# buaacyw/GaussianEditor

Hardware: AMD Instinct MI355X
Metric: train iters/sec (fwd+bwd of one 1080p view per GPU + grad all-reduce), 1M Gaussians @1080p (higher is better)
Workload: dtype f32; 1 GPU; synth-v1 1000000 Gaussians SH3 (M=16, s0=0.01), 1920x1080, ring-v1 8 views, one view per GPU (BASELINE.json configs[3] shape; configs[1] bicycle.ply is not available offline); gaussians=1000000, width=1920, height=1080, views_per_rank=1, parallelism=dp1-views, view_pipeline=False, tile_bounds=reference, fast_exp=False, grad_exchange=direct, grad_exchange_route=local, grad_rows=every row of every gradient written every iteration, num_rendered=0, visible=0, pixel_instances=0, sort_key_bits=45

## Files before the change

gaussianeditor_amd/_native.py:

```python
from __future__ import annotations

import ctypes
import os
from ctypes import c_float, c_int, c_int64, c_size_t, c_uint, c_void_p, POINTER

_HERE = os.path.dirname(os.path.abspath(__file__))
LIB_PATH = os.environ.get("GSR_LIBRARY_PATH") or os.path.join(_HERE, "libgsr_hip.so")
GSR_ABI_VERSION = 6

_P = c_void_p
ACC_ROW, ACC_MEAN2D, ACC_OPACITY, ACC_CONIC, ACC_COLOR, ACC_DEPTH = 16, 0, 3, 4, 8, 11


class AdamTensor(ctypes.Structure):
    _fields_ = [("param", _P), ("grad", _P), ("exp_avg", _P), ("exp_avg_sq", _P), ("anchor", _P), ("numel", c_int64),
                ("row_len", ctypes.c_int32), ("masked", ctypes.c_int32), ("lr", ctypes.c_double), ("anchor_scale", c_float)]


class DenseGrads(ctypes.Structure):
    _fields_ = [("means3D", _P), ("scales", _P), ("rotations", _P), ("means2D", _P), ("opacities", _P), ("sh", _P)]


class AppendTensor(ctypes.Structure):
    _fields_ = [("src", _P), ("ext", _P), ("dst", _P), ("row_bytes", c_int64)]
# ... 48 lines not shown
    "gsr_append_rows": (c_int, [_P, c_int64, c_int64, c_int, POINTER(AppendTensor)]),
    "gsr_adam_step": (c_int, [_P, c_int, POINTER(AdamTensor), c_int64, ctypes.c_double, ctypes.c_double, ctypes.c_double, _P,
                            _P]),
    "gsr_adam_step_rows": (c_int, [_P, c_int, POINTER(AdamTensor), c_int64, ctypes.c_double, ctypes.c_double, ctypes.c_double, _P,
                            _P, _P]),
    "gsr_mark_visible": (c_int, [_P, c_int, _P, _P, _P, _P]),
    "gsr_trace_weights": (c_int, [_P, c_int, c_int64, c_int, c_int, c_int, _P, _P, _P, _P, _P, _P, c_uint]),
    "gsr_debug_export_geom": (c_int, [_P, c_int, _P, _P, _P, _P, _P, _P, _P]),
    "gsr_debug_cov3d": (c_int, [_P, c_int, _P, c_float, _P, _P]),
    "gsr_debug_export_binning": (c_int, [_P, c_int, c_int64, c_int, c_int, _P, _P, _P, _P]),
    "gsr_debug_blend_backward_profile": (c_int, [_P, c_int, c_int64, c_int, c_int, _P, _P, _P, _P, _P, _P, _P,
                                                 c_int64, POINTER(c_int64)]),
    "gsr_debug_blend_forward_profile": (c_int, [_P, c_int, c_int64, c_int, c_int, _P, _P, _P, _P, _P, _P, _P, c_int64,
                                                POINTER(c_int64)]),
    "gsr_debug_export_image": (c_int, [_P, c_int, c_int, _P, _P, _P, _P]),
}

_lib = None


class GsrError(RuntimeError):

    def __init__(self, fn: str, status: int, message: str, hip_error: int = 0):
        self.status = status
        self.hip_error = hip_error
        extra = f" (hipError_t {hip_error})" if hip_error else ""
        super().__init__(f"{fn} failed: {message} [status {status}]{extra}")


def lib() -> ctypes.CDLL:
# ... 29 lines not shown
```

gaussianeditor_amd/csrc/gsr_binning.hip:

```cpp
#include <stdlib.h>

#include "gsr_kernels.h"

namespace gsr {

__device__ __forceinline__ int f2i_sat(float v) {
  if (!(v == v)) return 0;
  if (v >= 2147483648.0f) return 2147483647;
  if (v <= -2147483648.0f) return (-2147483647 - 1);
  return (int)v;
}

constexpr int RBITS = 8;
constexpr int RBINS = 1 << RBITS;

template <class K, int TH, bool WEIGHTED = false>
__global__ void __launch_bounds__(TH) sort_hist_kernel(const K* __restrict__ keys, int64_t n, int shift,
                                                                uint32_t mask, uint32_t* __restrict__ hist,
                                                                uint32_t nblocks, const uint4* __restrict__ publish_src,
                                                                uint32_t publish_count, uint32_t* __restrict__ publish_dst,
                                                                uint32_t publish_seq, const uint32_t* __restrict__ rect32) {
  __shared__ uint32_t h[RBINS];
  __shared__ uint32_t hw[WEIGHTED ? RBINS : 1];
  if (publish_dst != nullptr && blockIdx.x == nblocks) {
    __shared__ unsigned long long psum[TH / 64];
    __shared__ uint32_t pmax[TH / 64], pinv[TH / 64];
    __shared__ unsigned long long pgrp[TH / 64];
    unsigned long long sum = 0, gsum = 0;
    uint32_t kmax = 0, kinv = 0;
    constexpr int PUB_UNROLL = 8;
    for (uint32_t base = threadIdx.x; base < publish_count; base += TH * PUB_UNROLL) {
      uint4 v[PUB_UNROLL];
#pragma unroll
      for (int u = 0; u < PUB_UNROLL; ++u) v[u] = publish_src[min(base + (uint32_t)u * TH, publish_count - 1u)];
#pragma unroll
      for (int u = 0; u < PUB_UNROLL; ++u) {
        if (base + (uint32_t)u * TH < publish_count) {
          sum += v[u].x;
          gsum += v[u].w;
          kmax = max(kmax, v[u].y);
          kinv = max(kinv, v[u].z);
        }
      }
    }
#pragma unroll
    for (int d = 32; d >= 1; d >>= 1) {
      sum += __shfl_xor(sum, d, 64);
      gsum += __shfl_xor(gsum, d, 64);
      kmax = max(kmax, (uint32_t)__shfl_xor((int)kmax, d, 64));
      kinv = max(kinv, (uint32_t)__shfl_xor((int)kinv, d, 64));
    }
    if (lane_id() == 0) {
      psum[threadIdx.x >> 6] = sum;
      pgrp[threadIdx.x >> 6] = gsum;
      pmax[threadIdx.x >> 6] = kmax;
      pinv[threadIdx.x >> 6] = kinv;
    }
    __syncthreads();
    if (threadIdx.x == 0) {
      for (int w = 1; w < TH / 64; ++w) {
        sum += psum[w];
        gsum += pgrp[w];
        kmax = max(kmax, pmax[w]);
        kinv = max(kinv, pinv[w]);
      }
      publish_dst[0] = (uint32_t)sum;
      publish_dst[1] = (uint32_t)(sum >> 32);
      publish_dst[GEOM_HDR_KEYMAX] = kmax;
      publish_dst[GEOM_HDR_KEYINVMAX] = kinv;
      publish_dst[GEOM_HDR_GROUPS] = (uint32_t)gsum;
      publish_dst[GEOM_HDR_GROUPS + 1] = (uint32_t)(gsum >> 32);
      __threadfence_system();
      __hip_atomic_store(publish_dst + GEOM_HDR_FINAL, publish_seq, __ATOMIC_RELEASE, __HIP_MEMORY_SCOPE_SYSTEM);
    }
    return;
  }
  if (threadIdx.x < RBINS) {
    h[threadIdx.x] = 0;
    if (WEIGHTED) hw[threadIdx.x] = 0;
  }
  __syncthreads();
  const int64_t base = (int64_t)blockIdx.x * SORT_KPB;
  uint32_t kv[(SORT_KPB / TH)], rv[WEIGHTED ? (SORT_KPB / TH) : 1];
#pragma unroll
  for (int i = 0; i < (SORT_KPB / TH); ++i) {
    const int64_t k = base + (int64_t)i * TH + threadIdx.x;
    kv[i] = (uint32_t)keys[k < n ? k : n - 1];
    if (WEIGHTED) rv[i] = rect32[k < n ? k : n - 1];
  }
// ... 315 lines not shown
    const int j = i * TH + (int)threadIdx.x;
    if (j < nvalid) {
      const uint32_t kk = LAST ? 0u : skey[j];
      const uint32_t d = LAST ? (uint32_t)sdig[j] : (kk >> shift) & mask;
      const uint32_t first = lexcl[d];
      const uint32_t pos = gbase[d] + ((uint32_t)j - first);
      keys_out[pos] = LAST ? wgbase[d] + (spre[j] - spre[first]) : kk;
      vals_out[pos] = sval[j];
      rect_out[pos] = srect[j];
    }
  }
}

template <int TH>
static void depth_sort_grouped_th(hipStream_t s, int P, const Geom& g, int p0, int p1, bool last, uint32_t* publish_dst,
                                  uint32_t publish_seq) {
  const int64_t n = P;
  const uint32_t nblocks = (uint32_t)((n + SORT_KPB - 1) / SORT_KPB);
  const uint32_t npart = (uint32_t)((P + GAUSS_BLOCK - 1) / GAUSS_BLOCK);
  uint32_t* const hdr = reinterpret_cast<uint32_t*>(g.total);
  for (int p = p0; p < p1; ++p) {
    const int cur = p & 1, shift = 8 * p;
    const bool pub = p == p0 && publish_dst != nullptr, fin = last && p == p1 - 1;
    const dim3 gh(nblocks + (pub ? 1u : 0u)), gs(nblocks), bt(TH), bh(1024);
    if (fin)
      hipLaunchKernelGGL((sort_hist_kernel<uint32_t, 1024, true>), gh, bh, 0, s, (const uint32_t*)g.dkey[cur], n, shift, 255u, g.ghist,
                         nblocks, pub ? g.k1_partials : nullptr, npart, pub ? publish_dst : nullptr, publish_seq,
                         (const uint32_t*)g.drect[cur]);
    else
      hipLaunchKernelGGL((sort_hist_kernel<uint32_t, 1024, false>), gh, bh, 0, s, (const uint32_t*)g.dkey[cur], n, shift, 255u, g.ghist,
                         nblocks, pub ? g.k1_partials : nullptr, npart, pub ? publish_dst : nullptr, publish_seq,
                         (const uint32_t*)nullptr);
    hipLaunchKernelGGL(sort_scan_kernel, dim3(fin ? 2 * RBINS : RBINS), dim3(SORT_THREADS), 0, s, g.ghist, g.gbin_total, nblocks);
#define GSR_DEPTH_SCATTER(LASTP, IOTAP)                                                                                          \
  hipLaunchKernelGGL((depth_scatter_kernel<LASTP, IOTAP, TH>), gs, bt, 0, s, (const uint32_t*)g.dkey[cur],                       \
                     (const uint32_t*)g.dval[cur], (const uint32_t*)g.drect[cur], (const uint2*)g.rect, g.dkey[cur ^ 1],         \
                     g.dval[cur ^ 1], g.drect[cur ^ 1], n, shift, 255u, (const uint32_t*)g.ghist, (const uint32_t*)g.gbin_total, \
                     nblocks, hdr, (uint32_t)(cur ^ 1))
    if (fin && p == 0) GSR_DEPTH_SCATTER(true, true);
    else if (fin) GSR_DEPTH_SCATTER(true, false);
    else if (p == 0) GSR_DEPTH_SCATTER(false, true);
    else GSR_DEPTH_SCATTER(false, false);
#undef GSR_DEPTH_SCATTER
  }
}
hipError_t launch_depth_passes_grouped(hipStream_t s, int P, const Geom& g, int p0, int p1, bool last, uint32_t* publish_dst,
                                       uint32_t publish_seq) {
  if ((uint32_t)(((int64_t)P + SORT_KPB - 1) / SORT_KPB) <= SORT_WIDE_MAX_BLOCKS)
    depth_sort_grouped_th<1024>(s, P, g, p0, p1, last, publish_dst, publish_seq);
  else
    depth_sort_grouped_th<SORT_THREADS>(s, P, g, p0, p1, last, publish_dst, publish_seq);
  return hipGetLastError();
}

__global__ void __launch_bounds__(GAUSS_BLOCK) sorted_block_sums_kernel(int P, int gx, int sgx, const uint32_t* __restrict__ order,
                                                                       const uint2* __restrict__ rect,
                                                                       uint32_t* __restrict__ wh_sorted,
                                                                       uint32_t* __restrict__ org_sorted,
                                                                       uint32_t* __restrict__ block_sums,
                                                                       uint32_t* __restrict__ hdr, uint32_t final_buf) {
  __shared__ uint32_t smem[GAUSS_BLOCK / 64 + 1];
  if (blockIdx.x == 0 && threadIdx.x == 0) hdr[GEOM_HDR_FINAL] = final_buf;
  const int i = (int)(blockIdx.x * GAUSS_BLOCK + threadIdx.x);
  const uint2 rc = i < P ? rect[order[i]] : make_uint2(0u, 0u);
  const uint32_t w = rc.y & 0xffffu, h = rc.y >> 16, x0 = rc.x & 0xffffu, y0 = rc.x >> 16;
  uint32_t n = w * h, org = y0 * (uint32_t)gx + x0;
// ... 797 lines not shown
```

gaussianeditor_amd/csrc/gsr_capi.hip:

```cpp
#include <math.h>
#include <stdlib.h>
#include <string.h>

#include <chrono>
#include <mutex>


#include "gsr_kernels.h"

using namespace gsr;

namespace {
thread_local int g_last_hip_error = 0;
inline int hip_fail(hipError_t e) {
  g_last_hip_error = (int)e;
  return GSR_ERR_HIP;
}
#define GSR_HIP(expr)                          \
  do {                                         \
    hipError_t _e = (expr);                    \
    if (_e != hipSuccess) return hip_fail(_e); \
  } while (0)

struct HostSlot {
  uint32_t* words = nullptr;
  uint32_t* dev_words = nullptr;
  uint32_t seq = 0;
  int device = -1;
  HostSlot* next_free = nullptr;
};
constexpr int MAX_DEV = 64;
std::mutex g_pool_mutex;
HostSlot* g_pool_free[MAX_DEV] = {};

struct ThreadSlots {
  HostSlot* held[MAX_DEV] = {};
  ~ThreadSlots() {
    std::lock_guard<std::mutex> lock(g_pool_mutex);
    for (int d = 0; d < MAX_DEV; ++d)
      if (held[d] != nullptr) {
        held[d]->next_free = g_pool_free[d];
        g_pool_free[d] = held[d];
      }
// ... 131 lines not shown
}
inline bool geom_is_forward_only(const void* geom) {
  std::lock_guard<std::mutex> lock(g_notes_mutex);
  const GeomNote& n = g_notes[note_slot(geom)];
  return n.geom == geom && n.forward_only;
}

inline int bin_legacy(int W, int H) {
  static const bool forced = [] {
    const char* e = getenv("GSR_BIN_LEGACY");
    return e != nullptr && e[0] == '1';
  }();
  const int gx = (W + TILE - 1) / TILE, gy = (H + TILE - 1) / TILE;
  return (forced || group_count(W, H) > GROUP_MAX || gx > RECT32_EDGE || gy > RECT32_EDGE) ? 1 : 0;
}
inline int checkpoint_chunks(int64_t R, int W, int H) {
  static const int env = [] {
    const char* e = getenv("GSR_CK_CHUNKS");
    const char* d = getenv("GSR_CK_DEBUG");
    int c = e != nullptr ? atoi(e) : -1;
    if (c > 0 && c < 4 && !(d != nullptr && d[0] == '1')) c = 4;
    return c > 1024 ? 1024 : c;
  }();
  if (env >= 0) return env;
  static const int64_t env_min_list = [] {
    const char* e = getenv("GSR_CK_MIN_LIST");
    return (int64_t)(e != nullptr && atoi(e) > 0 ? atoi(e) : 0);
  }();
  const int64_t T = (int64_t)((W + TILE - 1) / TILE) * ((H + TILE - 1) / TILE);
  const int64_t min_list = env_min_list > 0 ? env_min_list : (T <= 4096 ? 1200 : 2048);
// ... 160 lines not shown
  a.opacities = opacities; a.shs = shs; a.cov3D_precomp = cov3D_precomp; a.colors_precomp = colors_precomp;
  a.viewmatrix = viewmatrix; a.projmatrix = projmatrix; a.campos = campos;
  a.W = W; a.H = H; a.tan_fovx = tan_fovx; a.tan_fovy = tan_fovy;
  a.focal_y = H / (2.0f * tan_fovy);
  a.focal_x = W / (2.0f * tan_fovx);
  a.gx = (W + TILE - 1) / TILE; a.gy = (H + TILE - 1) / TILE;
  a.skip_color = skip_color;
  a.forward_only = (flags & GSR_FLAG_FORWARD_ONLY) ? 1 : 0;
  a.tile_bounds = (flags & GSR_FLAG_TILE_BOUNDS_ALPHA) ? 1 : 0;
  a.radii = radii;
  a.g = carve_geom(geom, P);
  note_geom(geom, a.forward_only != 0);
  GSR_HIP(launch_preprocess(s, a));
  const uint32_t seq = ++slot->seq ? slot->seq : ++slot->seq;
  *seq_out = seq;
  if (bin_legacy(W, H)) GSR_HIP(launch_depth_passes(s, P, a.g, 0, 2, slot->dev_words, seq));
  else GSR_HIP(launch_depth_passes_grouped(s, P, a.g, 0, 2, false, slot->dev_words, seq));
  return GSR_OK;
}

int preprocess_end_impl(hipStream_t s, int P, int W, int H, void* geom, HostSlot* slot, uint32_t seq, int64_t counts_host[2]) {
  GSR_HIP(wait_for_slot(slot, seq, s));
  const Geom g = carve_geom(geom, P);
  const int gx = (W + TILE - 1) / TILE;
  const int legacy = bin_legacy(W, H);
  const uint32_t* w = slot->words;
  const uint64_t total = (uint64_t)w[0] | ((uint64_t)w[1] << 32);
  const uint32_t kmax = w[GEOM_HDR_KEYMAX], kinv = w[GEOM_HDR_KEYINVMAX];
  const uint32_t kmin = ~kinv;
  int nbits = 0;
  for (uint32_t d = total ? (kmax ^ kmin) : 0u; d; d >>= 1) ++nbits;
  if (legacy) {
    const int passes = nbits <= 16 ? 2 : (nbits + 7) / 8;
    if (passes > 2) GSR_HIP(launch_depth_passes(s, P, g, 2, passes));
    GSR_HIP(launch_depth_finish(s, P, g, passes, gx, 0));
  } else {
    const int passes = nbits <= 24 ? 3 : 4;
    GSR_HIP(launch_depth_passes_grouped(s, P, g, 2, passes, true));
  }
  if (total >= (1ull << 31)) return GSR_ERR_TOO_MANY;
  counts_host[0] = (int64_t)total;
  counts_host[1] = legacy ? 0 : (int64_t)((uint64_t)w[GEOM_HDR_GROUPS] | ((uint64_t)w[GEOM_HDR_GROUPS + 1] << 32));
  return GSR_OK;
}
}

int gsr_preprocess(void* stream, int P, int D, int M, const float* means3D, const float* scales, float scale_modifier,
                   const float* rotations, const float* opacities, const float* shs, const float* cov3D_precomp,
                   const float* colors_precomp, const float* viewmatrix, const float* projmatrix, const float* campos,
                   int W, int H, float tan_fovx, float tan_fovy, int prefiltered, int skip_color, unsigned flags,
// ... 584 lines not shown
}

int gsr_debug_export_binning(void* stream, int P, int64_t R, int W, int H, const void* geom, const void* binning,
                             uint64_t* keys, uint32_t* point_list) {
  if (R <= 0) return GSR_OK;
  if (!binning || !geom) return GSR_ERR_BAD_ARGUMENT;
  const Geom g = carve_geom(const_cast<void*>(geom), P);
  const Binning b = carve_binning_view(binning, R, W, H);
  hipStream_t s = (hipStream_t)stream;
  if (keys) GSR_HIP(launch_export_keys(s, R, W, H, b, g, keys));
  if (point_list)
    GSR_HIP(hipMemcpyAsync(point_list, b.point_list, sizeof(uint32_t) * (size_t)R, hipMemcpyDeviceToDevice, s));
  return GSR_OK;
}

int gsr_debug_export_image(void* stream, int W, int H, const void* image, uint32_t* ranges, float* final_T,
                           uint32_t* n_contrib) {
  if (!image || W <= 0 || H <= 0) return GSR_ERR_BAD_ARGUMENT;
  const Image im = carve_image(const_cast<void*>(image), W, H);
  hipStream_t s = (hipStream_t)stream;
  const size_t T = (size_t)((W + TILE - 1) / TILE) * ((H + TILE - 1) / TILE), N = (size_t)W * H;
  if (ranges) GSR_HIP(hipMemcpyAsync(ranges, im.ranges, sizeof(uint2) * T, hipMemcpyDeviceToDevice, s));
  if (final_T) GSR_HIP(hipMemcpyAsync(final_T, im.final_T, sizeof(float) * N, hipMemcpyDeviceToDevice, s));
  if (n_contrib) GSR_HIP(hipMemcpyAsync(n_contrib, im.n_contrib, sizeof(uint32_t) * N, hipMemcpyDeviceToDevice, s));
  return GSR_OK;
}

}
```

gaussianeditor_amd/csrc/gsr_common.h:

```cpp
#pragma once

#include <hip/hip_runtime.h>
#include <stddef.h>
#include <stdint.h>

#include "../../include/gsr.h"

namespace gsr {

constexpr int TILE = 16;
constexpr int QUAD = 8;
constexpr int WAVE = 64;
constexpr int GAUSS_BLOCK = 256;
constexpr uint32_t ACC_ROW = GSR_ACC_ROW, ACC_MEAN2D = GSR_ACC_MEAN2D, ACC_OPACITY = GSR_ACC_OPACITY, ACC_CONIC = GSR_ACC_CONIC,
                   ACC_COLOR = GSR_ACC_COLOR, ACC_DEPTH = GSR_ACC_DEPTH;
static_assert(ACC_ROW == 16 && ACC_MEAN2D == 0 && ACC_OPACITY == 3 && ACC_CONIC == 4 && ACC_COLOR == 8, "float4-aligned column groups");
static_assert(ACC_DEPTH == ACC_COLOR + 3, "the depth column is the .w of the colour group: K8+K9 reads it with the colour");
constexpr int GROUP_SHIFT = 3;
constexpr int GROUP_EDGE = 1 << GROUP_SHIFT;
constexpr int GROUP_TILES = GROUP_EDGE * GROUP_EDGE;
constexpr int GROUP_MAX = 2048;
constexpr uint32_t GROUP_PAD = 0xffffffffu;

__host__ __device__ inline size_t align_up(size_t v, size_t a = 256) { return (v + a - 1) / a * a; }
// ... 11 lines not shown
  uint4* k1_partials;
  uint32_t* dkey[2];
  uint32_t* dval[2];
  uint32_t* drect[2];
  uint32_t* ghist;
  uint32_t* gbin_total;
  size_t bytes;
};

constexpr int GEOM_HDR_SLOTS = 64;
constexpr int GEOM_HDR_SLOT_WORDS = 32;
constexpr int GEOM_HDR_KEYMAX = 2;
constexpr int GEOM_HDR_KEYINVMAX = 3;
constexpr int GEOM_HDR_FINAL = 4;
constexpr int GEOM_HDR_GROUPS = 5;
constexpr int GEOM_HDR_BYTES = GEOM_HDR_SLOTS * GEOM_HDR_SLOT_WORDS * 4;

__host__ __device__ inline Geom carve_geom(void* base, int P) {
  char* p = (char*)base;
  const size_t nb = ((size_t)P + GAUSS_BLOCK - 1) / GAUSS_BLOCK;
  Geom g;
  size_t off = 0;
  g.total = (uint64_t*)(p + off);      off += align_up(GEOM_HDR_BYTES);
  g.k1_partials = (uint4*)(p + off);   off += align_up(sizeof(uint4) * nb);
  g.rec0 = (float4*)(p + off);         off += align_up(sizeof(float4) * (size_t)P);
  g.rec1 = (float4*)(p + off);         off += align_up(sizeof(float4) * (size_t)P);
  g.rec2 = (float4*)(p + off);         off += align_up(sizeof(float4) * (size_t)P);
  for (int i = 0; i < 3; ++i) { g.dcol[i] = (float*)(p + off); off += align_up(sizeof(float) * 3 * (size_t)P); }
  g.rect = (uint2*)(p + off);          off += align_up(sizeof(uint2) * (size_t)P);
  g.clamped = (uint8_t*)(p + off);     off += align_up((size_t)P);
// ... 307 lines not shown
```

gaussianeditor_amd/csrc/gsr_kernels.h:

```cpp
#pragma once
#include "gsr_common.h"

namespace gsr {

struct PreArgs {
  int P, D, M;
  const float* means3D;
  const float* scales;
  float scale_modifier;
  const float* rotations;
  const float* opacities;
  const float* shs;
  const float* cov3D_precomp;
  const float* colors_precomp;
  const float* viewmatrix;
  const float* projmatrix;
  const float* campos;
  int W, H;
  float tan_fovx, tan_fovy, focal_x, focal_y;
  int gx, gy;
  int skip_color;
  int forward_only;
  int tile_bounds;
  int32_t* radii;
// ... 89 lines not shown
int64_t view_message_words_host(int64_t P, int64_t cap);
hipError_t launch_view_message_header(hipStream_t s, int64_t P, const float* campos, const uint32_t* block_off,
                                      const uint64_t* total, float* msg);
hipError_t launch_view_messages_accumulate(hipStream_t s, int64_t P, int D, int M, int n_views, const float* messages,
                                           int64_t stride_words, int64_t cap, const float* means3D, float* const dense[6],
                                           uint8_t* row_valid);
const uint32_t* compact_block_off_ptr(void* workspace, int64_t P);
hipError_t launch_export_cov3d(hipStream_t s, int P, const float* scales, float scale_modifier, const float* rotations,
                               float* cov3D);
hipError_t launch_export_geom(hipStream_t s, int P, const Geom& g, float* means2D, float* depths, float* rgb,
                              float* conic_opacity, uint32_t* tiles_touched, uint8_t* clamped);
hipError_t launch_depth_passes(hipStream_t s, int P, const Geom& g, int p0, int p1, uint32_t* publish_dst = nullptr,
                               uint32_t publish_seq = 0);
hipError_t launch_depth_finish(hipStream_t s, int P, const Geom& g, int passes, int gx, int sgx);
hipError_t launch_depth_passes_grouped(hipStream_t s, int P, const Geom& g, int p0, int p1, bool last,
                                       uint32_t* publish_dst = nullptr, uint32_t publish_seq = 0);
hipError_t launch_export_keys(hipStream_t s, int64_t R, int W, int H, const Binning& b, const Geom& g, uint64_t* keys);
hipError_t launch_binning(hipStream_t s, int P, int64_t R, int W, int H, const Geom& g, const Binning& b, const Image& im);
size_t knn_workspace_bytes(int P);
hipError_t launch_knn(hipStream_t s, int P, const float* points, void* workspace, float* out);
hipError_t launch_near_points(hipStream_t s, int n_ref, const float* ref, int n_query, const float* query, float thresh,
                              void* workspace, uint8_t* near, float* nn_dist);
size_t compact_workspace_bytes(int64_t P);
hipError_t launch_compact_plan(hipStream_t s, int64_t P, const uint8_t* keep, void* workspace);
const uint64_t* compact_total_ptr(void* workspace, int64_t P);
hipError_t launch_compact_apply(hipStream_t s, int64_t P, const uint8_t* keep, void* workspace, int nt,
                                const gsr_compact_tensor* tensors, int64_t limit = -1);
hipError_t launch_append_rows(hipStream_t s, int64_t P, int64_t n, int nt, const gsr_append_tensor* tensors);
hipError_t launch_adam_step(hipStream_t s, int nt, const gsr_adam_tensor* tensors, long long step, double beta1,
                            double beta2, double eps, const uint8_t* row_mask, const float* row_weight,
                            const uint8_t* grad_valid = nullptr);
// ... 7 lines not shown
```

include/gsr.h:

```cpp
#ifndef GSR_H_INCLUDED
#define GSR_H_INCLUDED

#include <stddef.h>
#include <stdint.h>

#ifdef __cplusplus
extern "C" {
#endif
#if defined(__GNUC__) || defined(__clang__)
#pragma GCC visibility push(default)
#endif

#define GSR_ABI_VERSION 6
#define GSR_ACC_ROW 16
#define GSR_ACC_MEAN2D 0
#define GSR_ACC_OPACITY 3
#define GSR_ACC_CONIC 4
#define GSR_ACC_COLOR 8
#define GSR_ACC_DEPTH 11
#define GSR_MAX_TILES (1 << 20)

typedef enum gsr_status {
  GSR_OK = 0,
  GSR_ERR_BAD_ARGUMENT = -1,
// ... 158 lines not shown
typedef struct gsr_append_tensor {
  const void* src;
  const void* ext;
  void* dst;
  int64_t row_bytes;
} gsr_append_tensor;
int gsr_append_rows(void* stream, int64_t P, int64_t n, int num_tensors, const gsr_append_tensor* tensors);

int gsr_debug_export_geom(void* stream, int P, const void* geom, float* means2D, float* depths, float* rgb,
                          float* conic_opacity, uint32_t* tiles_touched, uint8_t* clamped);
int gsr_debug_cov3d(void* stream, int P, const float* scales, float scale_modifier, const float* rotations, float* cov3D);
int gsr_debug_export_binning(void* stream, int P, int64_t R, int W, int H, const void* geom, const void* binning,
                             uint64_t* keys, uint32_t* point_list);
int gsr_debug_export_image(void* stream, int W, int H, const void* image, uint32_t* ranges, float* final_T,
                           uint32_t* n_contrib);

int gsr_debug_blend_backward_profile(void* stream, int P, int64_t R, int W, int H, const float* bg, const void* geom,
                                     const void* binning, const void* image, const float* dL_dpix, float* acc,
                                     uint64_t* records, int64_t max_records, int64_t* n_records_host);
int gsr_debug_blend_forward_profile(void* stream, int P, int64_t R, int W, int H, const float* bg, const void* geom,
                                    const void* binning, void* image, float* out_color, float* out_depth,
                                    uint64_t* records, int64_t max_records, int64_t* n_records_host);

#if defined(__GNUC__) || defined(__clang__)
#pragma GCC visibility pop
#endif
#ifdef __cplusplus
}
#endif
#endif
// ... 1 lines not shown
```

Measured before the change: 1800 view-iters/s.

## Replace multi-pass LSD depth radix sort with bucketed depth sort

Adds a depth-sort path that splits the float-key range into up to 256 linear buckets. A histogram pass and a scatter pass distribute Gaussians into buckets, then one block per bucket sorts its bucket in shared memory and writes the group prefix sums. This replaces the 3-4 grouped LSD radix passes, cutting global-memory round trips over the keys, values and rects. If any bucket exceeds the 16K shared-memory capacity, it falls back to grouped radix passes. The new path is on by default for P up to 2M and can be turned off with GSR_DEPTH_SORT=lsd.

```diff
diff --git a/gaussianeditor_amd/_native.py b/gaussianeditor_amd/_native.py
--- a/gaussianeditor_amd/_native.py
+++ b/gaussianeditor_amd/_native.py
@@ -86,6 +86,9 @@
     "gsr_debug_blend_forward_profile": (c_int, [_P, c_int, c_int64, c_int, c_int, _P, _P, _P, _P, _P, _P, _P, c_int64,
                                                 POINTER(c_int64)]),
     "gsr_debug_export_image": (c_int, [_P, c_int, c_int, _P, _P, _P, _P]),
+    "gsr_debug_export_depth_order": (c_int, [_P, c_int, _P, _P, _P, _P]),
+    "gsr_debug_set_depth_sort": (c_int, [c_int]),
+    "gsr_debug_depth_sort_path": (c_int, []),
 }
 
 _lib = None
diff --git a/gaussianeditor_amd/csrc/gsr_binning.hip b/gaussianeditor_amd/csrc/gsr_binning.hip
--- a/gaussianeditor_amd/csrc/gsr_binning.hip
+++ b/gaussianeditor_amd/csrc/gsr_binning.hip
@@ -13,6 +13,62 @@
 
 constexpr int RBITS = 8;
 constexpr int RBINS = 1 << RBITS;
+
+template <int TH>
+__device__ void publish_k1_counts(const uint4* __restrict__ publish_src, uint32_t publish_count,
+                                  uint32_t* __restrict__ publish_dst, uint32_t publish_seq) {
+  __shared__ unsigned long long psum[TH / 64];
+  __shared__ uint32_t pmax[TH / 64], pinv[TH / 64];
+  __shared__ unsigned long long pgrp[TH / 64];
+  unsigned long long sum = 0, gsum = 0;
+  uint32_t kmax = 0, kinv = 0;
+  constexpr int PUB_UNROLL = 8;
+  for (uint32_t base = threadIdx.x; base < publish_count; base += TH * PUB_UNROLL) {
+    uint4 v[PUB_UNROLL];
+#pragma unroll
+    for (int u = 0; u < PUB_UNROLL; ++u) v[u] = publish_src[min(base + (uint32_t)u * TH, publish_count - 1u)];
+#pragma unroll
+    for (int u = 0; u < PUB_UNROLL; ++u) {
+      if (base + (uint32_t)u * TH < publish_count) {
+        sum += v[u].x;
+        gsum += v[u].w;
+        kmax = max(kmax, v[u].y);
+        kinv = max(kinv, v[u].z);
+      }
+    }
+  }
+#pragma unroll
+  for (int d = 32; d >= 1; d >>= 1) {
+    sum += __shfl_xor(sum, d, 64);
+    gsum += __shfl_xor(gsum, d, 64);
+    kmax = max(kmax, (uint32_t)__shfl_xor((int)kmax, d, 64));
+    kinv = max(kinv, (uint32_t)__shfl_xor((int)kinv, d, 64));
+  }
+  if (lane_id() == 0) {
+    psum[threadIdx.x >> 6] = sum;
+    pgrp[threadIdx.x >> 6] = gsum;
+    pmax[threadIdx.x >> 6] = kmax;
+    pinv[threadIdx.x >> 6] = kinv;
+  }
+  __syncthreads();
+  if (threadIdx.x == 0) {
+    for (int w = 1; w < TH / 64; ++w) {
+      sum += psum[w];
+      gsum += pgrp[w];
+      kmax = max(kmax, pmax[w]);
+      kinv = max(kinv, pinv[w]);
+    }
+    publish_dst[0] = (uint32_t)sum;
+    publish_dst[1] = (uint32_t)(sum >> 32);
+    publish_dst[GEOM_HDR_KEYMAX] = kmax;
+    publish_dst[GEOM_HDR_KEYINVMAX] = kinv;
+    publish_dst[GEOM_HDR_GROUPS] = (uint32_t)gsum;
+    publish_dst[GEOM_HDR_GROUPS + 1] = (uint32_t)(gsum >> 32);
+    __threadfence_system();
+    if (publish_seq != 0u)
+      __hip_atomic_store(publish_dst + GEOM_HDR_FINAL, publish_seq, __ATOMIC_RELEASE, __HIP_MEMORY_SCOPE_SYSTEM);
+  }
+}
 
 template <class K, int TH, bool WEIGHTED = false>
 __global__ void __launch_bounds__(TH) sort_hist_kernel(const K* __restrict__ keys, int64_t n, int shift,
@@ -23,56 +79,7 @@
   __shared__ uint32_t h[RBINS];
   __shared__ uint32_t hw[WEIGHTED ? RBINS : 1];
   if (publish_dst != nullptr && blockIdx.x == nblocks) {
-    __shared__ unsigned long long psum[TH / 64];
-    __shared__ uint32_t pmax[TH / 64], pinv[TH / 64];
-    __shared__ unsigned long long pgrp[TH / 64];
-    unsigned long long sum = 0, gsum = 0;
-    uint32_t kmax = 0, kinv = 0;
-    constexpr int PUB_UNROLL = 8;
-    for (uint32_t base = threadIdx.x; base < publish_count; base += TH * PUB_UNROLL) {
-      uint4 v[PUB_UNROLL];
-#pragma unroll
-      for (int u = 0; u < PUB_UNROLL; ++u) v[u] = publish_src[min(base + (uint32_t)u * TH, publish_count - 1u)];
-#pragma unroll
-      for (int u = 0; u < PUB_UNROLL; ++u) {
-        if (base + (uint32_t)u * TH < publish_count) {
-          sum += v[u].x;
-          gsum += v[u].w;
-          kmax = max(kmax, v[u].y);
-          kinv = max(kinv, v[u].z);
-        }
-      }
-    }
-#pragma unroll
-    for (int d = 32; d >= 1; d >>= 1) {
-      sum += __shfl_xor(sum, d, 64);
-      gsum += __shfl_xor(gsum, d, 64);
-      kmax = max(kmax, (uint32_t)__shfl_xor((int)kmax, d, 64));
-      kinv = max(kinv, (uint32_t)__shfl_xor((int)kinv, d, 64));
-    }
-    if (lane_id() == 0) {
-      psum[threadIdx.x >> 6] = sum;
-      pgrp[threadIdx.x >> 6] = gsum;
-      pmax[threadIdx.x >> 6] = kmax;
-      pinv[threadIdx.x >> 6] = kinv;
-    }
-    __syncthreads();
-    if (threadIdx.x == 0) {
-      for (int w = 1; w < TH / 64; ++w) {
-        sum += psum[w];
-        gsum += pgrp[w];
-        kmax = max(kmax, pmax[w]);
-        kinv = max(kinv, pinv[w]);
-      }
-      publish_dst[0] = (uint32_t)sum;
-      publish_dst[1] = (uint32_t)(sum >> 32);
-      publish_dst[GEOM_HDR_KEYMAX] = kmax;
-      publish_dst[GEOM_HDR_KEYINVMAX] = kinv;
-      publish_dst[GEOM_HDR_GROUPS] = (uint32_t)gsum;
-      publish_dst[GEOM_HDR_GROUPS + 1] = (uint32_t)(gsum >> 32);
-      __threadfence_system();
-      __hip_atomic_store(publish_dst + GEOM_HDR_FINAL, publish_seq, __ATOMIC_RELEASE, __HIP_MEMORY_SCOPE_SYSTEM);
-    }
+    publish_k1_counts<TH>(publish_src, publish_count, publish_dst, publish_seq);
     return;
   }
   if (threadIdx.x < RBINS) {
@@ -418,13 +425,13 @@
 
 template <int TH>
 static void depth_sort_grouped_th(hipStream_t s, int P, const Geom& g, int p0, int p1, bool last, uint32_t* publish_dst,
-                                  uint32_t publish_seq) {
+                                  uint32_t publish_seq, int side0) {
   const int64_t n = P;
   const uint32_t nblocks = (uint32_t)((n + SORT_KPB - 1) / SORT_KPB);
   const uint32_t npart = (uint32_t)((P + GAUSS_BLOCK - 1) / GAUSS_BLOCK);
   uint32_t* const hdr = reinterpret_cast<uint32_t*>(g.total);
   for (int p = p0; p < p1; ++p) {
-    const int cur = p & 1, shift = 8 * p;
+    const int cur = (p & 1) ^ side0, shift = 8 * p;
     const bool pub = p == p0 && publish_dst != nullptr, fin = last && p == p1 - 1;
     const dim3 gh(nblocks + (pub ? 1u : 0u)), gs(nblocks), bt(TH), bh(1024);
     if (fin)
@@ -441,19 +448,447 @@
                      (const uint32_t*)g.dval[cur], (const uint32_t*)g.drect[cur], (const uint2*)g.rect, g.dkey[cur ^ 1],         \
                      g.dval[cur ^ 1], g.drect[cur ^ 1], n, shift, 255u, (const uint32_t*)g.ghist, (const uint32_t*)g.gbin_total, \
                      nblocks, hdr, (uint32_t)(cur ^ 1))
-    if (fin && p == 0) GSR_DEPTH_SCATTER(true, true);
+    if (fin && p == 0 && side0 == 0) GSR_DEPTH_SCATTER(true, true);
     else if (fin) GSR_DEPTH_SCATTER(true, false);
-    else if (p == 0) GSR_DEPTH_SCATTER(false, true);
+    else if (p == 0 && side0 == 0) GSR_DEPTH_SCATTER(false, true);
     else GSR_DEPTH_SCATTER(false, false);
 #undef GSR_DEPTH_SCATTER
   }
 }
 hipError_t launch_depth_passes_grouped(hipStream_t s, int P, const Geom& g, int p0, int p1, bool last, uint32_t* publish_dst,
-                                       uint32_t publish_seq) {
+                                       uint32_t publish_seq, int side0) {
   if ((uint32_t)(((int64_t)P + SORT_KPB - 1) / SORT_KPB) <= SORT_WIDE_MAX_BLOCKS)
-    depth_sort_grouped_th<1024>(s, P, g, p0, p1, last, publish_dst, publish_seq);
+    depth_sort_grouped_th<1024>(s, P, g, p0, p1, last, publish_dst, publish_seq, side0);
   else
-    depth_sort_grouped_th<SORT_THREADS>(s, P, g, p0, p1, last, publish_dst, publish_seq);
+    depth_sort_grouped_th<SORT_THREADS>(s, P, g, p0, p1, last, publish_dst, publish_seq, side0);
+  return hipGetLastError();
+}
+
+struct DepthBuckets {
+  uint32_t kmin;
+  uint32_t nb;
+  unsigned long long mul;
+};
+__device__ __forceinline__ DepthBuckets depth_buckets(uint32_t kmax, uint32_t kinv, uint32_t nb) {
+  DepthBuckets d;
+  d.nb = nb;
+  d.kmin = ~kinv;
+  d.mul = kmax >= d.kmin ? ((unsigned long long)nb << 32) / ((unsigned long long)(kmax - d.kmin) + 1ull) : 0ull;
+  return d;
+}
+__device__ __forceinline__ uint32_t depth_bucket(uint32_t key, const DepthBuckets& d) {
+  return key == 0xffffffffu ? d.nb : (uint32_t)(((unsigned long long)(key - d.kmin) * d.mul) >> 32);
+}
+
+constexpr int BUCKET_TH = 1024;
+
+__global__ void __launch_bounds__(BUCKET_TH) bucket_hist_kernel(const uint32_t* __restrict__ keys, const uint2* __restrict__ rect8,
+                                                                int64_t n, uint32_t nb, uint32_t* __restrict__ hist,
+                                                                uint32_t nblocks, const uint4* __restrict__ partials,
+                                                                uint32_t npart, uint32_t* __restrict__ publish_dst,
+                                                                uint32_t* __restrict__ hdr) {
+  constexpr int TH = BUCKET_TH, ITEMS = SORT_KPB / TH, NW = TH / 64;
+  __shared__ uint32_t h[RBINS], hw[RBINS];
+  __shared__ uint32_t smax[NW], sinv[NW];
+  if (blockIdx.x == nblocks) {
+    publish_k1_counts<TH>(partials, npart, publish_dst, 0u);
+    return;
+  }
+  const int64_t base = (int64_t)blockIdx.x * SORT_KPB;
+  uint32_t kv[ITEMS];
+  unsigned long long rv[ITEMS];
+#pragma unroll
+  for (int i = 0; i < ITEMS; ++i) {
+    const int64_t k = base + (int64_t)i * TH + threadIdx.x;
+    kv[i] = keys[k < n ? k : n - 1];
+    rv[i] = reinterpret_cast<const unsigned long long*>(rect8)[k < n ? k : n - 1];
+  }
+  if (threadIdx.x < RBINS) h[threadIdx.x] = hw[threadIdx.x] = 0u;
+  uint32_t kmax = 0u, kinv = 0u;
+  constexpr int UNROLL = 4;
+  for (uint32_t b = threadIdx.x; b < npart; b += TH * UNROLL) {
+    uint4 v[UNROLL];
+#pragma unroll
+    for (int u = 0; u < UNROLL; ++u) v[u] = partials[min(b + (uint32_t)u * TH, npart - 1u)];
+#pragma unroll
+    for (int u = 0; u < UNROLL; ++u) {
+      kmax = max(kmax, v[u].y);
+      kinv = max(kinv, v[u].z);
+    }
+  }
+#pragma unroll
+  for (int d = 32; d >= 1; d >>= 1) {
+    kmax = max(kmax, (uint32_t)__shfl_xor((int)kmax, d, 64));
+    kinv = max(kinv, (uint32_t)__shfl_xor((int)kinv, d, 64));
+  }
+  if (lane_id() == 0) {
+    smax[threadIdx.x >> 6] = kmax;
+    sinv[threadIdx.x >> 6] = kinv;
+  }
+  __syncthreads();
+#pragma unroll
+  for (int w = 0; w < NW; ++w) {
+    kmax = max(kmax, smax[w]);
+    kinv = max(kinv, sinv[w]);
+  }
+  if (blockIdx.x == 0 && threadIdx.x == 0) {
+    hdr[GEOM_HDR_DRANGE] = kmax;
+    hdr[GEOM_HDR_DRANGE + 1] = kinv;
+  }
+  const DepthBuckets db = depth_buckets(kmax, kinv, nb);
+#pragma unroll
+  for (int i = 0; i < ITEMS; ++i) {
+    const int64_t k = base + (int64_t)i * TH + threadIdx.x;
+    if (k < n && kv[i] != 0xffffffffu) {
+      const uint32_t d = depth_bucket(kv[i], db);
+      atomicAdd(&h[d], 1u);
+      const uint32_t g = rect32_groups(pack_rect32((uint32_t)rv[i], (uint32_t)(rv[i] >> 32)));
+      if (g != 0u) atomicAdd(&hw[d], g);
+    }
+  }
+  __syncthreads();
+  if (threadIdx.x < nb) {
+    hist[(size_t)threadIdx.x * nblocks + blockIdx.x] = h[threadIdx.x];
+    hist[(size_t)(nb + threadIdx.x) * nblocks + blockIdx.x] = hw[threadIdx.x];
+  }
+}
+
+constexpr int BBINS = RBINS + 1;
+__global__ void __launch_bounds__(BUCKET_TH) bucket_scatter_kernel(const Geom g, int64_t n, uint32_t nb,
+                                                                   const uint32_t* __restrict__ hist,
+                                                                   const uint32_t* __restrict__ bin_total, uint32_t nblocks,
+                                                                   uint32_t* __restrict__ publish_dst, uint32_t publish_seq) {
+  constexpr int TH = BUCKET_TH, NW = TH / 64, ITEMS = SORT_KPB / TH;
+  __shared__ uint32_t cnt[NW][BBINS];
+  __shared__ uint32_t gbase[BBINS], lexcl[BBINS];
+  __shared__ uint32_t smem[NW + 1];
+  __shared__ uint32_t sval[SORT_KPB], srect[SORT_KPB], skey[SORT_KPB];
+  __shared__ uint16_t sdig[SORT_KPB];
+  __shared__ uint32_t s_gtot;
+  const uint32_t* hdr = reinterpret_cast<const uint32_t*>(g.total);
+  const int w = (int)(threadIdx.x >> 6), l = lane_id();
+  const int64_t bbase = (int64_t)blockIdx.x * SORT_KPB;
+  const int64_t wbase = bbase + (int64_t)w * (ITEMS * 64);
+  uint32_t key[ITEMS], val[ITEMS], rc[ITEMS];
+  uint16_t rank[ITEMS];
+  const uint64_t lt_mask = (1ull << l) - 1ull;
+#pragma unroll
+  for (int i = 0; i < ITEMS; ++i) {
+    const int64_t k = wbase + (int64_t)i * 64 + l;
+    const int64_t kc = k < n ? k : n - 1;
+    key[i] = g.dkey[0][kc];
+    const unsigned long long r8 = reinterpret_cast<const unsigned long long*>(g.rect)[kc];
+    rc[i] = pack_rect32((uint32_t)r8, (uint32_t)(r8 >> 32));
+    val[i] = (uint32_t)kc;
+  }
+  const DepthBuckets db = depth_buckets(hdr[GEOM_HDR_DRANGE], hdr[GEOM_HDR_DRANGE + 1], nb);
+  const bool vis_bin = threadIdx.x < nb;
+  const uint32_t my_hist = vis_bin ? hist[(size_t)threadIdx.x * nblocks + blockIdx.x] : 0u;
+  const uint32_t my_total = vis_bin ? bin_total[threadIdx.x] : 0u;
+  const uint32_t my_wtotal = vis_bin ? bin_total[nb + threadIdx.x] : 0u;
+  for (int i = threadIdx.x; i < NW * BBINS; i += TH) (&cnt[0][0])[i] = 0;
+  {
+    uint32_t nvis, before_blk, gtot;
+    const uint32_t run = block_excl_scan_u32<TH>(my_total, &nvis, smem);
+    if (vis_bin) gbase[threadIdx.x] = run + my_hist;
+    (void)block_excl_scan_u32<TH>(my_hist, &before_blk, smem);
+    (void)block_excl_scan_u32<TH>(my_wtotal, &gtot, smem);
+    if (threadIdx.x == 0) {
+      gbase[nb] = nvis + ((uint32_t)bbase - before_blk);
+      s_gtot = gtot;
+    }
+    if (blockIdx.x == 0 && publish_dst != nullptr) {
+      uint32_t m = my_total;
+#pragma unroll
+      for (int d = 32; d >= 1; d >>= 1) m = max(m, (uint32_t)__shfl_xor((int)m, d, 64));
+      __syncthreads();
+      if (l == 0) smem[w] = m;
+      __syncthreads();
+      if (threadIdx.x == 0) {
+        for (int i = 1; i < NW; ++i) m = max(m, smem[i]);
+        publish_dst[GEOM_HDR_BUCKETMAX] = m;
+        __threadfence_system();
+        __hip_atomic_store(publish_dst + GEOM_HDR_FINAL, publish_seq, __ATOMIC_RELEASE, __HIP_MEMORY_SCOPE_SYSTEM);
+      }
+    }
+  }
+  __syncthreads();
+
+  uint32_t dig[ITEMS];
+#pragma unroll
+  for (int i = 0; i < ITEMS; ++i) {
+    const int64_t k = wbase + (int64_t)i * 64 + l;
+    const bool valid = k < n;
+    const uint32_t d = depth_bucket(key[i], db);
+    dig[i] = d;
+    uint64_t m = __ballot(valid);
+#pragma unroll
+    for (int b = 0; b < RBITS + 1; ++b) {
+      const uint64_t bb = __ballot((d >> b) & 1u);
+      m &= ((d >> b) & 1u) ? bb : ~bb;
+    }
+    const uint32_t before = (uint32_t)__popcll(m & lt_mask);
+    uint32_t old = 0;
+    if (valid) old = cnt[w][d];
+    if (valid && before == 0) cnt[w][d] = old + (uint32_t)__popcll(m);
+    rank[i] = (uint16_t)(old + before);
+  }
+  __syncthreads();
+  {
+    const bool owns = threadIdx.x <= nb;
+    uint32_t run = 0;
+    if (owns) {
+#pragma unroll
+      for (int i = 0; i < NW; ++i) {
+        const uint32_t c = cnt[i][threadIdx.x];
+        cnt[i][threadIdx.x] = run;
+        run += c;
+      }
+    }
+    uint32_t tot;
+    const uint32_t ex = block_excl_scan_u32<TH>(run, &tot, smem);
+    if (owns) lexcl[threadIdx.x] = ex;
+  }
+  __syncthreads();
+#pragma unroll
+  for (int i = 0; i < ITEMS; ++i) {
+    const int64_t k = wbase + (int64_t)i * 64 + l;
+    if (k < n) {
+      const uint32_t d = dig[i];
+      const uint32_t lp = lexcl[d] + cnt[w][d] + rank[i];
+      sdig[lp] = (uint16_t)d;
+      skey[lp] = key[i];
+      sval[lp] = val[i];
+      srect[lp] = rc[i];
+    }
+  }
+  __syncthreads();
+  const int nvalid = (int)min((int64_t)SORT_KPB, n - bbase);
+  const uint32_t gtot = s_gtot;
+#pragma unroll
+  for (int i = 0; i < ITEMS; ++i) {
+    const int j = i * TH + (int)threadIdx.x;
+    if (j < nvalid) {
+      const uint32_t d = sdig[j];
+      const uint32_t pos = gbase[d] + ((uint32_t)j - lexcl[d]);
+      g.dkey[1][pos] = skey[j];
+      g.dval[1][pos] = sval[j];
+      g.drect[1][pos] = srect[j];
+      if (d == nb) {
+        g.dkey[0][pos] = gtot;
+        g.dval[0][pos] = sval[j];
+        g.drect[0][pos] = srect[j];
+      }
+    }
+  }
+}
+
+constexpr int BUCKET_ITEMS = (int)DEPTH_BUCKET_CAP / BUCKET_TH;
+static_assert(DEPTH_BUCKET_CAP <= 65536u && BUCKET_ITEMS * BUCKET_TH == (int)DEPTH_BUCKET_CAP, "bucket slots are 16 bits");
+__global__ void __launch_bounds__(BUCKET_TH) bucket_sort_kernel(const Geom g, uint32_t nb, const uint32_t* __restrict__ bin_total) {
+  constexpr int TH = BUCKET_TH, NW = TH / 64, ITEMS = BUCKET_ITEMS;
+  __shared__ uint32_t skey[DEPTH_BUCKET_CAP];
+  __shared__ uint16_t sli[DEPTH_BUCKET_CAP];
+  __shared__ uint32_t cnt[NW][RBINS];
+  __shared__ uint32_t lexcl[RBINS];
+  __shared__ uint32_t smem[NW + 1], sred[2][NW];
+  __shared__ uint32_t s_start, s_n, s_wbase, s_max;
+  uint32_t* const hdr = reinterpret_cast<uint32_t*>(g.total);
+  const int w = (int)(threadIdx.x >> 6), l = lane_id();
+  const uint32_t b = blockIdx.x;
+  {
+    const uint32_t c = threadIdx.x < nb ? bin_total[threadIdx.x] : 0u;
+    const uint32_t wc = threadIdx.x < nb ? bin_total[nb + threadIdx.x] : 0u;
+    uint32_t tot;
+    const uint32_t ex = block_excl_scan_u32<TH>(c, &tot, smem);
+    const uint32_t wex = block_excl_scan_u32<TH>(wc, &tot, smem);
+    uint32_t m = c;
+#pragma unroll
+    for (int d = 32; d >= 1; d >>= 1) m = max(m, (uint32_t)__shfl_xor((int)m, d, 64));
+    if (l == 0) sred[0][w] = m;
+    if (threadIdx.x == b) {
+      s_start = ex;
+      s_n = c;
+      s_wbase = wex;
+    }
+    __syncthreads();
+    if (threadIdx.x == 0) {
+      for (int i = 1; i < NW; ++i) m = max(m, sred[0][i]);
+      s_max = m;
+    }
+    __syncthreads();
+  }
+  if (s_max > DEPTH_BUCKET_CAP) return;
+  if (b == 0 && threadIdx.x == 0) hdr[GEOM_HDR_FINAL] = 0u;
+  const uint32_t n = s_n, start = s_start, wbase_g = s_wbase;
+  if (n == 0u) return;
+  const uint32_t chunk = ((n + TH - 1u) / TH) * 64u, iters = chunk / 64u;
+  const uint32_t base = (uint32_t)w * chunk;
+  const uint64_t lt_mask = (1ull << l) - 1ull;
+  uint32_t key[ITEMS], li[ITEMS];
+  uint16_t rank[ITEMS];
+  uint32_t kmin = 0xffffffffu, kmax = 0u;
+#pragma unroll
+  for (int i = 0; i < ITEMS; ++i) {
+    const uint32_t p = base + (uint32_t)i * 64u + (uint32_t)l;
+    li[i] = p;
+    key[i] = g.dkey[1][start + min(p, n - 1u)];
+  }
+#pragma unroll
+  for (int i = 0; i < ITEMS; ++i) {
+    if ((uint32_t)i < iters && li[i] < n) {
+      kmin = min(kmin, key[i]);
+      kmax = max(kmax, key[i]);
+    }
+  }
+#pragma unroll
+  for (int d = 32; d >= 1; d >>= 1) {
+    kmin = min(kmin, (uint32_t)__shfl_xor((int)kmin, d, 64));
+    kmax = max(kmax, (uint32_t)__shfl_xor((int)kmax, d, 64));
+  }
+  if (l == 0) {
+    sred[0][w] = kmin;
+    sred[1][w] = kmax;
+  }
+  __syncthreads();
+#pragma unroll
+  for (int i = 0; i < NW; ++i) {
+    kmin = min(kmin, sred[0][i]);
+    kmax = max(kmax, sred[1][i]);
+  }
+  int rbits = 0;
+  for (uint32_t d = kmax - kmin; d; d >>= 1) ++rbits;
+  const int passes = (rbits + RBITS - 1) / RBITS;
+#pragma unroll
+  for (int i = 0; i < ITEMS; ++i) key[i] -= kmin;
+
+  for (int pass = 0; pass < passes; ++pass) {
+    const int shift = pass * RBITS;
+    for (int i = threadIdx.x; i < NW * RBINS; i += TH) (&cnt[0][0])[i] = 0u;
+    __syncthreads();
+#pragma unroll
+    for (int i = 0; i < ITEMS; ++i) {
+      if ((uint32_t)i < iters) {
+        const bool valid = base + (uint32_t)i * 64u + (uint32_t)l < n;
+        const uint32_t d = (key[i] >> shift) & (RBINS - 1u);
+        uint64_t m = __ballot(valid);
+#pragma unroll
+        for (int bit = 0; bit < RBITS; ++bit) {
+          const uint64_t bb = __ballot((d >> bit) & 1u);
+          m &= ((d >> bit) & 1u) ? bb : ~bb;
+        }
+        const uint32_t before = (uint32_t)__popcll(m & lt_mask);
+        uint32_t old = 0;
+        if (valid) old = cnt[w][d];
+        if (valid && before == 0) cnt[w][d] = old + (uint32_t)__popcll(m);
+        rank[i] = (uint16_t)(old + before);
+      }
+    }
+    __syncthreads();
+    {
+      const bool owns = threadIdx.x < RBINS;
+      uint32_t run = 0;
+      if (owns) {
+#pragma unroll
+        for (int i = 0; i < NW; ++i) {
+          const uint32_t c = cnt[i][threadIdx.x];
+          cnt[i][threadIdx.x] = run;
+          run += c;
+        }
+      }
+      uint32_t tot;
+      const uint32_t ex = block_excl_scan_u32<TH>(run, &tot, smem);
+      if (owns) lexcl[threadIdx.x] = ex;
+    }
+    __syncthreads();
+#pragma unroll
+    for (int i = 0; i < ITEMS; ++i) {
+      if ((uint32_t)i < iters && base + (uint32_t)i * 64u + (uint32_t)l < n) {
+        const uint32_t d = (key[i] >> shift) & (RBINS - 1u);
+        const uint32_t lp = lexcl[d] + cnt[w][d] + rank[i];
+        skey[lp] = key[i];
+        sli[lp] = (uint16_t)li[i];
+      }
+    }
+    __syncthreads();
+#pragma unroll
+    for (int i = 0; i < ITEMS; ++i) {
+      const uint32_t p = base + (uint32_t)i * 64u + (uint32_t)l;
+      key[i] = skey[p];
+      li[i] = sli[p];
+    }
+  }
+  uint32_t v[ITEMS], r[ITEMS];
+#pragma unroll
+  for (int i = 0; i < ITEMS; ++i) {
+    const uint32_t p = base + (uint32_t)i * 64u + (uint32_t)l;
+    v[i] = g.dval[1][start + min(p, n - 1u)];
+    r[i] = g.drect[1][start + min(p, n - 1u)];
+  }
+  if (passes > 0) {
+    __syncthreads();
+#pragma unroll
+    for (int i = 0; i < ITEMS; ++i) {
+      const uint32_t p = base + (uint32_t)i * 64u + (uint32_t)l;
+      if ((uint32_t)i < iters && p < n) skey[p] = v[i];
+    }
+    __syncthreads();
+#pragma unroll
+    for (int i = 0; i < ITEMS; ++i) {
+      const uint32_t p = base + (uint32_t)i * 64u + (uint32_t)l;
+      if ((uint32_t)i < iters && p < n) v[i] = skey[li[i]];
+    }
+    __syncthreads();
+#pragma unroll
+    for (int i = 0; i < ITEMS; ++i) {
+      const uint32_t p = base + (uint32_t)i * 64u + (uint32_t)l;
+      if ((uint32_t)i < iters && p < n) skey[p] = r[i];
+    }
+    __syncthreads();
+#pragma unroll
+    for (int i = 0; i < ITEMS; ++i) {
+      const uint32_t p = base + (uint32_t)i * 64u + (uint32_t)l;
+      if ((uint32_t)i < iters && p < n) r[i] = skey[li[i]];
+    }
+  }
+  uint32_t pre[ITEMS], run = 0;
+#pragma unroll
+  for (int i = 0; i < ITEMS; ++i) {
+    pre[i] = 0u;
+    if ((uint32_t)i < iters) {
+      const uint32_t gi = base + (uint32_t)i * 64u + (uint32_t)l < n ? rect32_groups(r[i]) : 0u;
+      const uint32_t incl = wave_incl_scan_dpp(gi);
+      pre[i] = run + incl - gi;
+      run += (uint32_t)__shfl((int)incl, 63, 64);
+    }
+  }
+  if (l == 0) smem[w] = run;
+  __syncthreads();
+  uint32_t wex = wbase_g;
+  for (int i = 0; i < w; ++i) wex += smem[i];
+#pragma unroll
+  for (int i = 0; i < ITEMS; ++i) {
+    const uint32_t p = base + (uint32_t)i * 64u + (uint32_t)l;
+    if ((uint32_t)i < iters && p < n) {
+      g.dkey[0][start + p] = wex + pre[i];
+      g.dval[0][start + p] = v[i];
+      g.drect[0][start + p] = r[i];
+    }
+  }
+}
+
+hipError_t launch_depth_buckets(hipStream_t s, int P, const Geom& g, uint32_t* publish_dst, uint32_t publish_seq) {
+  const int64_t n = P;
+  const uint32_t nblocks = (uint32_t)((n + SORT_KPB - 1) / SORT_KPB);
+  const uint32_t npart = (uint32_t)((P + GAUSS_BLOCK - 1) / GAUSS_BLOCK);
+  const uint32_t nb = (uint32_t)min((int64_t)RBINS, max((int64_t)1, (n + SORT_KPB - 1) / SORT_KPB));
+  hipLaunchKernelGGL(bucket_hist_kernel, dim3(nblocks + 1), dim3(BUCKET_TH), 0, s, (const uint32_t*)g.dkey[0],
+                     (const uint2*)g.rect, n, nb, g.ghist, nblocks, (const uint4*)g.k1_partials, npart, publish_dst,
+                     reinterpret_cast<uint32_t*>(g.total));
+  hipLaunchKernelGGL(sort_scan_kernel, dim3(2 * nb), dim3(SORT_THREADS), 0, s, g.ghist, g.gbin_total, nblocks);
+  hipLaunchKernelGGL(bucket_scatter_kernel, dim3(nblocks), dim3(BUCKET_TH), 0, s, g, n, nb, (const uint32_t*)g.ghist,
+                     (const uint32_t*)g.gbin_total, nblocks, publish_dst, publish_seq);
+  hipLaunchKernelGGL(bucket_sort_kernel, dim3(nb), dim3(BUCKET_TH), 0, s, g, nb, (const uint32_t*)g.gbin_total);
   return hipGetLastError();
 }
 
diff --git a/gaussianeditor_amd/csrc/gsr_capi.hip b/gaussianeditor_amd/csrc/gsr_capi.hip
--- a/gaussianeditor_amd/csrc/gsr_capi.hip
+++ b/gaussianeditor_amd/csrc/gsr_capi.hip
@@ -2,6 +2,7 @@
 #include <stdlib.h>
 #include <string.h>
 
+#include <atomic>
 #include <chrono>
 #include <mutex>
 
@@ -27,6 +28,7 @@
   uint32_t* dev_words = nullptr;
   uint32_t seq = 0;
   int device = -1;
+  bool depth_buckets = false;
   HostSlot* next_free = nullptr;
 };
 constexpr int MAX_DEV = 64;
@@ -188,6 +190,16 @@
   const int gx = (W + TILE - 1) / TILE, gy = (H + TILE - 1) / TILE;
   return (forced || group_count(W, H) > GROUP_MAX || gx > RECT32_EDGE || gy > RECT32_EDGE) ? 1 : 0;
 }
+std::atomic<int> g_depth_sort_override{-1};
+thread_local int g_last_depth_path = -1;
+inline bool depth_sort_buckets(int P) {
+  static const bool lsd = [] {
+    const char* e = getenv("GSR_DEPTH_SORT");
+    return e != nullptr && strcmp(e, "lsd") == 0;
+  }();
+  const int forced = g_depth_sort_override.load(std::memory_order_relaxed);
+  return P <= DEPTH_BUCKET_MAX_P && (forced >= 0 ? forced == 1 : !lsd);
+}
 inline int checkpoint_chunks(int64_t R, int W, int H) {
   static const int env = [] {
     const char* e = getenv("GSR_CK_CHUNKS");
@@ -378,7 +390,9 @@
   GSR_HIP(launch_preprocess(s, a));
   const uint32_t seq = ++slot->seq ? slot->seq : ++slot->seq;
   *seq_out = seq;
+  slot->depth_buckets = !bin_legacy(W, H) && depth_sort_buckets(P);
   if (bin_legacy(W, H)) GSR_HIP(launch_depth_passes(s, P, a.g, 0, 2, slot->dev_words, seq));
+  else if (slot->depth_buckets) GSR_HIP(launch_depth_buckets(s, P, a.g, slot->dev_words, seq));
   else GSR_HIP(launch_depth_passes_grouped(s, P, a.g, 0, 2, false, slot->dev_words, seq));
   return GSR_OK;
 }
@@ -394,10 +408,17 @@
   const uint32_t kmin = ~kinv;
   int nbits = 0;
   for (uint32_t d = total ? (kmax ^ kmin) : 0u; d; d >>= 1) ++nbits;
+  g_last_depth_path = 0;
   if (legacy) {
     const int passes = nbits <= 16 ? 2 : (nbits + 7) / 8;
     if (passes > 2) GSR_HIP(launch_depth_passes(s, P, g, 2, passes));
     GSR_HIP(launch_depth_finish(s, P, g, passes, gx, 0));
+  } else if (slot->depth_buckets) {
+    g_last_depth_path = 1;
+    if (w[GEOM_HDR_BUCKETMAX] > DEPTH_BUCKET_CAP) {
+      GSR_HIP(launch_depth_passes_grouped(s, P, g, 0, nbits > 8 ? (nbits + 7) / 8 : 1, true, nullptr, 0, 1));
+      g_last_depth_path = 2;
+    }
   } else {
     const int passes = nbits <= 24 ? 3 : 4;
     GSR_HIP(launch_depth_passes_grouped(s, P, g, 2, passes, true));
@@ -1012,6 +1033,30 @@
   return GSR_OK;
 }
 
+int gsr_debug_export_depth_order(void* stream, int P, const void* geom, uint32_t* order, uint32_t* rect, uint32_t* prefix) {
+  if (P <= 0) return GSR_OK;
+  if (!geom || misaligned(geom)) return GSR_ERR_BAD_ARGUMENT;
+  const Geom g = carve_geom(const_cast<void*>(geom), P);
+  hipStream_t s = (hipStream_t)stream;
+  uint32_t fin = 0;
+  GSR_HIP(hipMemcpyAsync(&fin, reinterpret_cast<const uint32_t*>(g.total) + GEOM_HDR_FINAL, sizeof(fin), hipMemcpyDeviceToHost, s));
+  GSR_HIP(hipStreamSynchronize(s));
+  if (fin > 1u) return GSR_ERR_BAD_ARGUMENT;
+  const size_t bytes = sizeof(uint32_t) * (size_t)P;
+  if (order) GSR_HIP(hipMemcpyAsync(order, g.dval[fin], bytes, hipMemcpyDeviceToDevice, s));
+  if (rect) GSR_HIP(hipMemcpyAsync(rect, g.drect[fin], bytes, hipMemcpyDeviceToDevice, s));
+  if (prefix) GSR_HIP(hipMemcpyAsync(prefix, g.dkey[fin], bytes, hipMemcpyDeviceToDevice, s));
+  return GSR_OK;
+}
+
+int gsr_debug_set_depth_sort(int mode) {
+  if (mode < -1 || mode > 1) return GSR_ERR_BAD_ARGUMENT;
+  g_depth_sort_override.store(mode, std::memory_order_relaxed);
+  return GSR_OK;
+}
+
+int gsr_debug_depth_sort_path(void) { return g_last_depth_path; }
+
 int gsr_debug_export_image(void* stream, int W, int H, const void* image, uint32_t* ranges, float* final_T,
                            uint32_t* n_contrib) {
   if (!image || W <= 0 || H <= 0) return GSR_ERR_BAD_ARGUMENT;
diff --git a/gaussianeditor_amd/csrc/gsr_common.h b/gaussianeditor_amd/csrc/gsr_common.h
--- a/gaussianeditor_amd/csrc/gsr_common.h
+++ b/gaussianeditor_amd/csrc/gsr_common.h
@@ -49,6 +49,8 @@
 constexpr int GEOM_HDR_KEYINVMAX = 3;
 constexpr int GEOM_HDR_FINAL = 4;
 constexpr int GEOM_HDR_GROUPS = 5;
+constexpr int GEOM_HDR_BUCKETMAX = 7;
+constexpr int GEOM_HDR_DRANGE = 10;
 constexpr int GEOM_HDR_BYTES = GEOM_HDR_SLOTS * GEOM_HDR_SLOT_WORDS * 4;
 
 __host__ __device__ inline Geom carve_geom(void* base, int P) {
diff --git a/gaussianeditor_amd/csrc/gsr_kernels.h b/gaussianeditor_amd/csrc/gsr_kernels.h
--- a/gaussianeditor_amd/csrc/gsr_kernels.h
+++ b/gaussianeditor_amd/csrc/gsr_kernels.h
@@ -127,7 +127,10 @@
                                uint32_t publish_seq = 0);
 hipError_t launch_depth_finish(hipStream_t s, int P, const Geom& g, int passes, int gx, int sgx);
 hipError_t launch_depth_passes_grouped(hipStream_t s, int P, const Geom& g, int p0, int p1, bool last,
-                                       uint32_t* publish_dst = nullptr, uint32_t publish_seq = 0);
+                                       uint32_t* publish_dst = nullptr, uint32_t publish_seq = 0, int side0 = 0);
+constexpr int DEPTH_BUCKET_MAX_P = 1 << 21;
+constexpr uint32_t DEPTH_BUCKET_CAP = 16384;
+hipError_t launch_depth_buckets(hipStream_t s, int P, const Geom& g, uint32_t* publish_dst, uint32_t publish_seq);
 hipError_t launch_export_keys(hipStream_t s, int64_t R, int W, int H, const Binning& b, const Geom& g, uint64_t* keys);
 hipError_t launch_binning(hipStream_t s, int P, int64_t R, int W, int H, const Geom& g, const Binning& b, const Image& im);
 size_t knn_workspace_bytes(int P);
diff --git a/include/gsr.h b/include/gsr.h
--- a/include/gsr.h
+++ b/include/gsr.h
@@ -196,6 +196,9 @@
                              uint64_t* keys, uint32_t* point_list);
 int gsr_debug_export_image(void* stream, int W, int H, const void* image, uint32_t* ranges, float* final_T,
                            uint32_t* n_contrib);
+int gsr_debug_export_depth_order(void* stream, int P, const void* geom, uint32_t* order, uint32_t* rect, uint32_t* prefix);
+int gsr_debug_set_depth_sort(int mode);
+int gsr_debug_depth_sort_path(void);
 
 int gsr_debug_blend_backward_profile(void* stream, int P, int64_t R, int W, int H, const float* bg, const void* geom,
                                      const void* binning, const void* image, const float* dL_dpix, float* acc,
```

Result: no change. 1813 view-iters/s (median of 4 runs) (+0.7%).
